# IvanPopov/video-flow-ml

Measured on AMD Instinct MI355X. Metric: flow-fields/sec @1080p seq5 MOF_sintel, higher is better.
Workload: dtype mixed (per-layer MFMA count, f32 accumulate): {"corr": 1, "update_block.encoder.convf1": 1, "update_block.encoder.convf2": 1, "update_block.gru.convq1.iter": "2a", "update_block.gru.convzr1.iter": 1, "update_block.gru.convzr2.iter": 1, "update_block.mask.0": 1, "update_block.mask.2": 1, "update_bloc

## Files before the change

video-flow-ml_amd/vfml/csrc/conv_gemm_split.hip:

```cpp
#include "conv_split_common.h"
#include "gemm_resident_walk.h"

namespace {

template <int BN, int WM, int WN, bool BIGC, bool IN16, int NM = 3>
__global__ __launch_bounds__(WM * WN * 64, 2) void conv_gemm_split_kernel(const SplitArgs a) {
  constexpr bool ALO = NM == 3 || NM == 2, BLO = NM == 3 || NM == 4;
  constexpr int NT = WM * WN * 64;
  constexpr int LR = NT / 4;
  constexpr int TM = BM / (WM * 32);
  constexpr int TN = BN / (WN * 32);
  constexpr int AU = BM / LR;
  constexpr int BU = BN / LR;
  constexpr int BUN = BU > 0 ? BU : 1;
  constexpr int RSA = BM + 2;
  constexpr int RSB = BN + 2;
  constexpr int SA = KG * RSA;
  constexpr int SB = KG * RSB;
  constexpr int LDC = BN + 4;

  extern __shared__ __attribute__((aligned(16))) char smem_raw[];
  h16x8* sAh = reinterpret_cast<h16x8*>(smem_raw);
  h16x8* sAl = sAh + 2 * SA;
  h16x8* sBh = sAl + 2 * SA;
// ... 154 lines not shown
    for (int j = 0; j < TN; ++j)
#pragma unroll
      for (int e = 0; e < 16; ++e) acc[i][j][e] = 0.f;

  auto compute = [&](int buf) {
    const int oa = buf * SA + wm * (BM / WM) + r;
    const int ob = buf * SB + wn * (BN / WN) + r;
#pragma unroll
    for (int ks = 0; ks < KG / 2; ++ks) {
      h16x8 ah[TM], al[TM], bh[TN], bl[TN];
#pragma unroll
      for (int i = 0; i < TM; ++i) {
        ah[i] = sAh[oa + (2 * ks + half) * RSA + i * 32];
        if constexpr (ALO) al[i] = sAl[oa + (2 * ks + half) * RSA + i * 32];
      }
#pragma unroll
      for (int j = 0; j < TN; ++j) {
        bh[j] = sBh[ob + (2 * ks + half) * RSB + j * 32];
        if constexpr (BLO) bl[j] = sBl[ob + (2 * ks + half) * RSB + j * 32];
      }
#pragma unroll
      for (int i = 0; i < TM; ++i)
#pragma unroll
        for (int j = 0; j < TN; ++j) {
          acc[i][j] = __builtin_amdgcn_mfma_f32_32x32x16_f16(ah[i], bh[j], acc[i][j], 0, 0, 0);
          if constexpr (BLO) acc[i][j] = __builtin_amdgcn_mfma_f32_32x32x16_f16(ah[i], bl[j], acc[i][j], 0, 0, 0);
          if constexpr (ALO) acc[i][j] = __builtin_amdgcn_mfma_f32_32x32x16_f16(al[i], bh[j], acc[i][j], 0, 0, 0);
        }
    }
  };

  const int nk = ((a.K + BK - 1) / BK + 1) & ~1;
  load_tile(st0, 0);
  load_tile(st1, BK);
  store_tile(st0, 0);
  __syncthreads();
  for (int kt = 0; kt < nk; kt += 2) {
    load_tile(st0, (kt + 2) * BK);
    __builtin_amdgcn_sched_barrier(0);
    compute(0);
    __builtin_amdgcn_sched_barrier(0);
    store_tile(st1, 1);
    __syncthreads();
    load_tile(st1, (kt + 3) * BK);
    __builtin_amdgcn_sched_barrier(0);
    compute(1);
    __builtin_amdgcn_sched_barrier(0);
    store_tile(st0, 0);
    __syncthreads();
  }

  acc_to_lds<TM, TN, LDC>(acc, sC, wm * (BM / WM), wn * (BN / WN), r, half);
  __syncthreads();
  if (!epilogue_rows_fast<BN, NT>(a, sC, m0, n0, t, BM, 32, 0)) epilogue_rows<BN, NT>(a, sC, m0, n0, t);
  if (a.stats_part) {
    constexpr int RG = NT / BN;
    const int ch = t % BN, rg = t / BN;
    double s1 = 0.0, s2 = 0.0;
    if (n0 + ch < a.cout) {
      const float b = a.bias ? a.bias[n0 + ch] : 0.f;
      for (int row = rg; row < BM; row += RG) {
        if (m0 + row >= a.M) break;
        const double v = (double)((sC[row * LDC + ch] * a.w_inv + b) * a.out_scale);
        s1 += v;
        s2 += v * v;
      }
    }
    __syncthreads();
    double* fold = reinterpret_cast<double*>(sC);
    fold[(rg * BN + ch) * 2] = s1;
    fold[(rg * BN + ch) * 2 + 1] = s2;
    __syncthreads();
    if (rg == 0 && n0 + ch < a.cout) {
      for (int g = 1; g < RG; ++g) {
        s1 += vfml_lds_f64(&fold[(g * BN + ch) * 2]);
        s2 += vfml_lds_f64(&fold[(g * BN + ch) * 2 + 1]);
      }
      double* o = a.stats_part + ((int64_t)(m0 / BM) * a.cout + n0 + ch) * 2;
      o[0] = s1;
      o[1] = s2;
    }
  }
}



template <int TM, int TN, int WM, int WN, bool PERSIST, bool FASTK, bool CSWAP = false, int NM = 3, bool MF16 = false, bool H16 = false>
__global__ __launch_bounds__(WM * WN * 64, (WM * WN == 4 ? 2 : 1)) void conv_gemm_dma_kernel(const SplitArgs a) {
  static_assert(!H16 || PERSIST, "VFML_FMT_F16 outputs (H16) exist in the persistent GEMM form only");
  static_assert(!(MF16 && PERSIST), "the persistent GEMM form runs 32x32x16 MFMAs (its 16x16x32 epilogue branches below are not maintained)");
  constexpr bool H64 = NM == 5;
  static_assert(!H64 || FASTK, "64-channel steps exist for the uniform-step loader only");
  constexpr bool BHI = NM == 2 || NM == 1 || H64;
  constexpr bool AHI = NM == 4 || NM == 1 || H64;
  constexpr int KSTEP = H64 ? 64 : BK;
  constexpr int NW = WM * WN, NT = NW * 64;
  constexpr int TBM = 32 * TM * WM, TBN = 32 * TN * WN;
  constexpr int AP = TBM / (8 * NW), BP = TBN / (8 * NW);
  static_assert(TBM % (8 * NW) == 0 && TBN % (8 * NW) == 0, "tile rows must split into whole pieces per wave");
  constexpr int ASZ = TBM * 128, BSZ = TBN * 128, STG = ASZ + BSZ;
  constexpr int LDC = TBN + 4;

  extern __shared__ __attribute__((aligned(16))) char smem_raw[];
  float* sC = reinterpret_cast<float*>(smem_raw);

  if constexpr (PERSIST && FASTK && !CSWAP && NM == 5 && !MF16) {
    if (a.resident) {
// ... 419 lines not shown
          }
        }
        if constexpr (PERSIST && TN == 2 && FASTK) if (a.out_t) {
          if constexpr (MF16) {
            static_for<2>([&](auto tc) {
              constexpr int t2 = decltype(tc)::value;
              static_for<2 * TN>([&](auto jc) {
                constexpr int j = decltype(jc)::value;
#pragma unroll
                for (int e = 0; e < 4; ++e) {
                  float v = 0.f;
                  static_for<TM>([&](auto ii) { if (decltype(ii)::value == i) v = acc4[2 * decltype(ii)::value + t2][j][e]; });
                  const int row = t2 * 16 + 4 * u4 + e, col = j * 16 + r4;
                  ws[col * 32 + ((row + (col >> 1)) & 31)] = v;
                }
              });
            });
          } else {
#pragma unroll
          for (int j = 0; j < TN; ++j)
#pragma unroll
            for (int e = 0; e < 16; ++e) {
              const int row = (e & 3) + 8 * (e >> 2) + 4 * half, col = j * 32 + r;
              ws[col * 32 + ((row + (col >> 1)) & 31)] = acc[i][j][e];
            }
          }
          const int rows_t = cols_valid, cols_t = rows_valid;
          char* tbase_t = reinterpret_cast<char*>(cur_ks ? a.out_t_k1 : a.out_t) + ((int64_t)cur_n0 * a.ld_out_t + cur_m0) * ES;
          const __amdgpu_buffer_rsrc_t rt =
              __builtin_amdgcn_make_buffer_rsrc(tbase_t, 0, ((rows_t - 1) * a.ld_out_t + cols_t) * ES, 0x00020000);
          const int g = lane >> 3, cl = lane & 7;
#pragma unroll
          for (int pp = 0; pp < 8; ++pp) {
            const int c = pp * 8 + cl;
            f32x4 v;
#pragma unroll
            for (int k = 0; k < 4; ++k) v[k] = ws[c * 32 + ((4 * g + k + (c >> 1)) & 31)] * a.w_inv * a.out_scale;
            const int q0 = wm * (32 * TM) + i * 32 + 4 * g;
            const int trow = wn * WC + c;
            const bool ok = trow < rows_t && q0 < cols_t;
            if constexpr (H16) {
              const h16x2 p0 = {(_Float16)v[0], (_Float16)v[1]}, p1 = {(_Float16)v[2], (_Float16)v[3]};
              const u32x2 hv = {__builtin_bit_cast(unsigned, p0), __builtin_bit_cast(unsigned, p1)};
              __builtin_amdgcn_raw_buffer_store_b64(hv, rt, ok ? (trow * a.ld_out_t + q0) * 2 : OOB, 0, STORE_NT);
            } else {
              __builtin_amdgcn_raw_buffer_store_b128(__builtin_bit_cast(u32x4, v), rt,
                                                     ok ? (trow * a.ld_out_t + q0) * 4 : OOB, 0, STORE_NT);
            }
          }
        }
      }
      stores_behind = true;
    } else {
      {
      static_for<TM>([&](auto slab) {
        constexpr int i = decltype(slab)::value;
        __syncthreads();
        if constexpr (PROJ && i == 0) {
          if (a.proj_out) proj_weights_store(pw, smem_raw + proj_lds_off<TBN>(), t);
        }
        if constexpr (MF16) {
          static_for<2>([&](auto tc) {
            constexpr int t2 = decltype(tc)::value;
            static_for<2 * TN>([&](auto jc) {
              constexpr int j = decltype(jc)::value;
              f32x4 v = {0.f, 0.f, 0.f, 0.f};
              static_for<TM>([&](auto ii) { if (decltype(ii)::value == i) v = acc4[2 * decltype(ii)::value + t2][j]; });
              *reinterpret_cast<f32x4*>(&sC[(wm * 32 + t2 * 16 + r4) * LDC + wn * (32 * TN) + j * 16 + 4 * u4]) = v;
            });
          });
        } else {
#pragma unroll
        for (int j = 0; j < TN; ++j)
#pragma unroll
          for (int e = 0; e < 16; ++e) {
            const int row = wm * 32 + (e & 3) + 8 * (e >> 2) + 4 * half;
            const int col = wn * (32 * TN) + j * 32 + r;
            sC[row * LDC + col] = acc[i][j][e];
          }
        }
        __syncthreads();
        bool projected = false;
        if constexpr (PROJ) {
          if (a.proj_out) {
            epilogue_proj_slab<TBN, NT, NM == 4>(a, sC, cur_m0, cur_n0, t, WM * 32, 32 * TM, i * 32);
            projected = true;
          }
        }
        if (!projected && !epilogue_rows_fast<TBN, NT>(a, sC, cur_m0, cur_n0, t, WM * 32, 32 * TM, i * 32))
          epilogue_rows<TBN, NT>(a, sC, cur_m0, cur_n0, t, WM * 32, 32 * TM, i * 32);
        if (a.stats_part) {
          for (int p = t; p < TBN * WM; p += NT) {
            const int ch = p % TBN, wb = p / TBN;
            const int g0 = cur_m0 + wb * (32 * TM) + i * 32;
            if (cur_n0 + ch < a.cout && g0 < a.M) {
              const float b = a.bias ? a.bias[cur_n0 + ch] : 0.f;
              double s1 = 0.0, s2 = 0.0;
              for (int rr = 0; rr < 32; ++rr) {
                if (g0 + rr >= a.M) break;
                const double v = (double)((sC[(wb * 32 + rr) * LDC + ch] * a.w_inv + b) * a.out_scale);
                s1 += v;
                s2 += v * v;
              }
              double* o = a.stats_part + ((int64_t)(g0 >> 5) * a.cout + cur_n0 + ch) * 2;
              o[0] = s1;
              o[1] = s2;
            }
          }
        }
      });
      }
    }
    if (!PERSIST || next >= tile_end) break;
    tile = next;
  }
}


template <int TM, int TN, int WM, int WN, bool PERSIST, bool FASTK, bool CSWAP = false, int NM = 3, bool MF16 = false, bool H16 = false>
int launch_dma_k(SplitArgs& a, hipStream_t s) {
  constexpr int TBM = 32 * TM * WM, TBN = 32 * TN * WN;
  constexpr size_t stage = 2 * (size_t)(TBM + TBN) * 128;
  constexpr size_t slab = (size_t)WM * 32 * (TBN + 4) * 4;
  constexpr size_t lds = (PERSIST || stage > slab) ? stage : slab;
  static_assert(lds <= 160 * 1024, "LDS");
  a.mtiles = (a.M + TBM - 1) / TBM;
  a.ntiles = (a.cout + TBN - 1) / TBN;
  constexpr bool HAS_RESIDENT = PERSIST && FASTK && !CSWAP && NM == 5 && !MF16;
  constexpr size_t lds_resident = VFML_RESIDENT_LDS;
  if (const int rc = vfml_lds_cap(reinterpret_cast<const void*>(&conv_gemm_dma_kernel<TM, TN, WM, WN, PERSIST, FASTK, CSWAP, NM, MF16, H16>),
                                  (int)(HAS_RESIDENT && lds_resident > lds ? lds_resident : lds), "vfml_conv2d_split"))
    return rc;
  if (a.resident) {
    if (!HAS_RESIDENT) {
      vfml_set_error("vfml_conv2d_split: the plan asks for the resident-A walk of a kernel that has none");
      return 1;
    }
    a.mtiles = (a.M + 127) / 128;
    a.ntiles = (a.cout + 63) / 64;
    int64_t best = -1;
    for (int nc = 1; nc <= a.ntiles && nc <= 512; ++nc) {
      const int cl = (a.ntiles + nc - 1) / nc, runs = (a.ntiles + cl - 1) / cl;
      const int64_t cost = (((int64_t)a.mtiles * runs + 511) / 512) * (cl + 3);
      if (best < 0 || cost < best) {
        best = cost;
        a.res_cl = cl;
        a.res_nc = runs;
      }
    }
    const int64_t units = (int64_t)a.mtiles * a.res_nc;
    hipLaunchKernelGGL((conv_gemm_dma_kernel<TM, TN, WM, WN, PERSIST, FASTK, CSWAP, NM, MF16, H16>), dim3((int)(units > 512 ? 512 : units)),
                       dim3(WM * WN * 64), lds_resident, s, a);
    return vfml_check_launch("vfml_conv2d_split");
  }
  const int64_t total = (int64_t)a.mtiles * a.ntiles * (PERSIST ? a.ksplit : 1);
  const int64_t slots = 256 * (WM * WN == 4 ? 2 : 1);
  const int grid = (int)(PERSIST && total > slots ? slots : total);
  hipLaunchKernelGGL((conv_gemm_dma_kernel<TM, TN, WM, WN, PERSIST, FASTK, CSWAP, NM, MF16, H16>), dim3(grid), dim3(WM * WN * 64), lds, s, a);
  return vfml_check_launch("vfml_conv2d_split");
}

template <int BN, int WM, int WN, bool BIGC, bool IN16, int NM>
int launch_nm(SplitArgs& a, hipStream_t s) {
// ... 646 lines not shown
```

video-flow-ml_amd/vfml/csrc/conv_gemm_tapx.hip:

```cpp
#include "conv_split_common.h"

#ifndef VFML_TAPX_HOOKS
#define TAPX_HOOK_ENTRY()
#define TAPX_HOOK_KLOOP_BEGIN()
#define TAPX_HOOK_STEP_BEGIN(st)
#define TAPX_HOOK_STAMP(k)
#define TAPX_HOOK_STEP_END()
#define TAPX_HOOK_KLOOP_END(nsteps)
#define TAPX_HOOK_EXIT()
#endif

namespace {

template <int TM, int TN, int WM, int WN, int NM>
__global__ __launch_bounds__(256, 2) void conv_gemm_tapx_kernel(const SplitArgs a) {
  constexpr bool H64 = NM == 5;
  constexpr bool BHI = NM == 2 || NM == 1 || H64;
  constexpr bool AHI = NM == 4 || NM == 1 || H64;
  constexpr int KSTEP = H64 ? 64 : 32;
  constexpr int NT = 256;
  static_assert(WM * WN == 4, "four waves: two workgroups per CU");
  constexpr int TBM = 32 * TM * WM, TBN = 32 * TN * WN;
  constexpr int NPA = (TBM + VFML_TAPX_KWMAX - 1 + 7) / 8;
  constexpr int NPI = (NPA + 3) / 4;
// ... 127 lines not shown
      const int R0 = r4 + kx;
      const int swa = (R0 >> 1) & 7;
      const int aoffk = abuf + (wm * (32 * TM) + R0) * 128 + (H64 ? (u4 ^ swa) : ((2 * u4) ^ swz16(swa))) * 16;
      auto a_addr = [&](int i) { return (unsigned)(oxp[i] + kx) < (unsigned)a.W ? aoffk + i * 2048 : ZOFF; };
      h16x8 a0, a1;
      {
        const int ad = a_addr(0);
        a0 = *reinterpret_cast<const h16x8*>(smem_raw + ad);
        if constexpr (H64 || !AHI) a1 = *reinterpret_cast<const h16x8*>(smem_raw + (ad ^ X1));
      }
      __syncthreads();
      TAPX_HOOK_STAMP(1);
      __builtin_amdgcn_sched_barrier(0);
      static_for<2 * TM>([&](auto ic) {
        constexpr int i = decltype(ic)::value;
        h16x8 n0_, n1_;
        if constexpr (i + 1 < 2 * TM) {
          const int ad = a_addr(i + 1);
          n0_ = *reinterpret_cast<const h16x8*>(smem_raw + ad);
          if constexpr (H64 || !AHI) n1_ = *reinterpret_cast<const h16x8*>(smem_raw + (ad ^ X1));
        }
        static_for<2 * TN>([&](auto jc) {
          constexpr int j = decltype(jc)::value;
          acc4[i][j] = __builtin_amdgcn_mfma_f32_16x16x32_f16(b0[j], a0, acc4[i][j], 0, 0, 0);
          if constexpr (H64) {
            acc4[i][j] = __builtin_amdgcn_mfma_f32_16x16x32_f16(b1[j], a1, acc4[i][j], 0, 0, 0);
          } else {
            if constexpr (!BHI) acc4[i][j] = __builtin_amdgcn_mfma_f32_16x16x32_f16(b1[j], a0, acc4[i][j], 0, 0, 0);
            if constexpr (!AHI) acc4[i][j] = __builtin_amdgcn_mfma_f32_16x16x32_f16(b0[j], a1, acc4[i][j], 0, 0, 0);
          }
          constexpr int g = i * (2 * TN) + j;
          if constexpr (g < BP) {
            if (next_step) issue_b(g, st + 1);
          } else if constexpr (g < BP + ASLOTS) {
            const int ia = kx + (g - BP) * a.kw;
            if (next_stage && ia < NPI && 4 * ia + wave < NPA) issue_a(ia, nbuf, cbn, kyn);
          }
          __builtin_amdgcn_sched_barrier(0);
        });
        if constexpr (i + 1 < 2 * TM) {
          a0 = n0_;
          if constexpr (H64 || !AHI) a1 = n1_;
        }
      });
      TAPX_HOOK_STAMP(2);
      asm volatile("s_waitcnt vmcnt(0)" ::: "memory");
      TAPX_HOOK_STAMP(3);
      __syncthreads();
      TAPX_HOOK_STEP_END();
    }
  }

  TAPX_HOOK_KLOOP_END(nsteps);
#pragma unroll
  for (int i = 0; i < TM; ++i) {
    if (i) lds_barrier();
    static_for<2>([&](auto tc) {
      constexpr int t2 = decltype(tc)::value;
      static_for<2 * TN>([&](auto jc) {
        constexpr int j = decltype(jc)::value;
        f32x4 v = {0.f, 0.f, 0.f, 0.f};
        static_for<TM>([&](auto ii) { if (decltype(ii)::value == i) v = acc4[2 * decltype(ii)::value + t2][j]; });
        *reinterpret_cast<f32x4*>(&sC[(wm * 32 + t2 * 16 + r4) * LDC + wn * (32 * TN) + j * 16 + 4 * u4]) = v;
      });
    });
    lds_barrier();
    if (!epilogue_rows_fast<TBN, NT>(a, sC, m0, n0, t, WM * 32, 32 * TM, i * 32))
      epilogue_rows<TBN, NT>(a, sC, m0, n0, t, WM * 32, 32 * TM, i * 32);
    if (a.stats_part) {
      for (int p = t; p < TBN * WM; p += NT) {
        const int ch = p % TBN, wb = p / TBN;
        const int g0 = m0 + wb * (32 * TM) + i * 32;
        if (n0 + ch < a.cout && g0 < a.M) {
          const float b = a.bias ? a.bias[n0 + ch] : 0.f;
          double s1 = 0.0, s2 = 0.0;
          for (int rr = 0; rr < 32; ++rr) {
            if (g0 + rr >= a.M) break;
            const double v = (double)((sC[(wb * 32 + rr) * LDC + ch] * a.w_inv + b) * a.out_scale);
            s1 += v;
            s2 += v * v;
          }
          double* o = a.stats_part + ((int64_t)(g0 >> 5) * a.cout + n0 + ch) * 2;
          o[0] = s1;
          o[1] = s2;
        }
      }
    }
  }
  TAPX_HOOK_EXIT();
}

template <int TM, int TN, int WM, int WN, int NM>
int launch_tapx_k(SplitArgs& a, hipStream_t s) {
  constexpr int TBM = 32 * TM * WM, TBN = 32 * TN * WN;
  constexpr int NPA = (TBM + VFML_TAPX_KWMAX - 1 + 7) / 8;
  constexpr size_t stage = 2 * (size_t)NPA * 1024 + (size_t)TBN * 128 + 128;
  constexpr size_t slab = (size_t)WM * 32 * (TBN + 4) * 4;
  constexpr size_t lds = stage > slab ? stage : slab;
  static_assert(lds <= 80 * 1024, "two workgroups per CU");
  a.mtiles = (a.M + TBM - 1) / TBM;
  a.ntiles = (a.cout + TBN - 1) / TBN;
  if (const int rc = vfml_lds_cap(reinterpret_cast<const void*>(&conv_gemm_tapx_kernel<TM, TN, WM, WN, NM>), (int)lds,
                                  "vfml_conv2d_split"))
    return rc;
  hipLaunchKernelGGL((conv_gemm_tapx_kernel<TM, TN, WM, WN, NM>), dim3(a.mtiles * a.ntiles), dim3(256), lds, s, a);
  return vfml_check_launch("vfml_conv2d_split");
}

#define TAPX_ROWS(TM, TN, WM, WN) \
  {vfml_detail::tapx_plan(TM, TN, WM, WN, 3), &launch_tapx_k<TM, TN, WM, WN, 3>}, \
  {vfml_detail::tapx_plan(TM, TN, WM, WN, 5), &launch_tapx_k<TM, TN, WM, WN, 5>}
const SplitVariant TAPX_VARIANTS[] = {TAPX_ROWS(3, 2, 2, 2), TAPX_ROWS(2, 3, 2, 2), TAPX_ROWS(2, 2, 4, 1), TAPX_ROWS(2, 3, 4, 1)};
#undef TAPX_ROWS

}

const SplitVariant* vfml_detail::tapx_variant(const SplitPlan& plan) {
  return find_variant(TAPX_VARIANTS, sizeof(TAPX_VARIANTS) / sizeof(TAPX_VARIANTS[0]), plan);
}

const SplitVariant* vfml_detail::tapx_variant_at(int index) {
  const int n = (int)(sizeof(TAPX_VARIANTS) / sizeof(TAPX_VARIANTS[0]));
  return index >= 0 && index < n ? &TAPX_VARIANTS[index] : nullptr;
}
```

video-flow-ml_amd/vfml/csrc/conv_split_common.h:

```cpp
#pragma once
#include <hip/hip_fp16.h>
#include <stdlib.h>
#include <utility>
#include "vfml_common.h"


namespace vfml_detail {
struct SplitArgs {
  const float* in0; const float* in1;
  const _Float16* whi; const _Float16* wlo; const float* bias;
  const float* aux0; const float* aux1; const float* addend;
  float* out;
  int c0, ld0, c1, ld1, ctot, ld_addend;
  int H, W, ho, wo;
  int kh, kw, stride, pad_h, pad_w;
  int M, K, Kp, cout;
  int d0off, d1off;
  int bytes0, bytesw;
  int ldo, ld_aux0, ld_aux1;
  int epilogue, split;
  float out_scale, w_inv;
  int mtiles, ntiles;
  int vec_ok;
  int out16, aux16;
// ... 189 lines not shown
      if (nvalid == 4) {
        if (epi == VFML_EPI_GRU_ZR && !lowhalf) x0 = aux4(a.aux0, a.ld_aux0, grow, col - a.split);
        if (epi == VFML_EPI_GRU_Q) {
          x0 = aux4(a.aux0, a.ld_aux0, grow, col);
          x1 = aux4(a.aux1, a.ld_aux1, grow, col);
        }
        if (epi == VFML_EPI_ADD_AUX) x0 = aux4(a.aux0, a.ld_aux0, grow, col);
      } else {
        for (int e = 0; e < nvalid; ++e) {
          if (epi == VFML_EPI_GRU_ZR && !lowhalf) x0[e] = a.aux0[(int64_t)grow * a.ld_aux0 + col + e - a.split];
          if (epi == VFML_EPI_GRU_Q) {
            x0[e] = a.aux0[(int64_t)grow * a.ld_aux0 + col + e];
            x1[e] = a.aux1[(int64_t)grow * a.ld_aux1 + col + e];
          }
          if (epi == VFML_EPI_ADD_AUX) x0[e] = a.aux0[(int64_t)grow * a.ld_aux0 + col + e];
        }
      }
#pragma unroll
      for (int e = 0; e < 4; ++e) v[e] = epi1(v[e], epi, lowhalf, x0[e], x1[e]);
      if (a.out16) {
        U8 hi, lo;
        split4(v, hi, lo, 0);
        char* u = reinterpret_cast<char*>(a.out + (int64_t)grow * a.ldo + gcol) + 8 * q;
        *reinterpret_cast<uint2*>(u) = __builtin_bit_cast(uint2, __builtin_shufflevector(hi.v, hi.v, 0, 1, 2, 3));
        *reinterpret_cast<uint2*>(u + 16) = __builtin_bit_cast(uint2, __builtin_shufflevector(lo.v, lo.v, 0, 1, 2, 3));
      } else {
        float* o = a.out + (int64_t)grow * a.ldo + col;
        if (nvalid == 4 && a.vec_ok) {
          *reinterpret_cast<f32x4*>(o) = v;
        } else {
          for (int e = 0; e < nvalid; ++e) o[e] = v[e];
        }
      }
    }
  }
}

template <int EPI>
__device__ __forceinline__ void epi_unit(f32x4 (&v)[2], const f32x4 (&x0)[2], const f32x4 (&x1)[2], bool lowhalf) {
#pragma unroll
  for (int q = 0; q < 2; ++q)
#pragma unroll
    for (int e = 0; e < 4; ++e) {
      float r = v[q][e];
      if constexpr (EPI == VFML_EPI_RELU) r = fmaxf(r, 0.f);
      else if constexpr (EPI == VFML_EPI_TANH) r = tanhf(r);
      else if constexpr (EPI == VFML_EPI_SIGMOID) r = sigmoidf_(r);
      else if constexpr (EPI == VFML_EPI_GRU_ZR) { r = sigmoidf_(r); r = lowhalf ? r : r * x0[q][e]; }
      else if constexpr (EPI == VFML_EPI_GRU_Q) r = (1.f - x0[q][e]) * x1[q][e] + x0[q][e] * tanhf(r);
      v[q][e] = r;
    }
}

__device__ __forceinline__ void load_unit16(const float* base, int64_t off, f32x4 (&x)[2]) {
  const h16x8 h = *reinterpret_cast<const h16x8*>(base + off);
  const h16x8 l = *reinterpret_cast<const h16x8*>(base + off + 4);
#pragma unroll
  for (int e = 0; e < 8; ++e) x[e >> 2][e & 3] = (float)h[e] + (float)l[e];
}

template <int BN, int NT, int EPI>
__device__ __forceinline__ void epilogue_rows_fast_k(const SplitArgs& a, const float* sC, int m0, int n0, int t, int nrows,
                                                     int rstride, int roff) {
  constexpr int LDC = BN + 4;
  constexpr int C8 = BN / 8;
  constexpr int RPP = NT / C8;
  if constexpr (NT % C8 != 0) {
    if (t >= RPP * C8) return;
  }
  const int c8 = t % C8;
  const int gcol = n0 + c8 * 8;
  if (gcol >= a.cout) return;
  const bool whole = gcol + 8 <= a.cout;
  f32x4 bias4[2] = {{0.f, 0.f, 0.f, 0.f}, {0.f, 0.f, 0.f, 0.f}};
  if (a.bias) {
    bias4[0] = *reinterpret_cast<const f32x4*>(a.bias + gcol);
    if (whole) bias4[1] = *reinterpret_cast<const f32x4*>(a.bias + gcol + 4);
  }
  const bool lowhalf = gcol < a.split;
  const vfml_gfptr addend = addend_of(a);
  struct RowOps {
    f32x4 add[2], x0[2], x1[2];
  };
  auto load_row = [&](int row, RowOps& o) {
    const int grow = m0 + (row >> 5) * rstride + roff + (row & 31);
    o.add[0] = o.add[1] = f32x4{0.f, 0.f, 0.f, 0.f};
    o.x0[0] = o.x0[1] = o.x1[0] = o.x1[1] = f32x4{0.f, 0.f, 0.f, 0.f};
    if (row >= nrows || grow >= a.M) return;
    if (a.addend) {
      o.add[0] = *(vfml_gf4ptr)(addend + (int64_t)grow * a.ld_addend + gcol);
      if (whole) o.add[1] = *(vfml_gf4ptr)(addend + (int64_t)grow * a.ld_addend + gcol + 4);
    }
    if constexpr (EPI == VFML_EPI_GRU_ZR) {
      if (!lowhalf) load_unit16(a.aux0, (int64_t)grow * a.ld_aux0 + gcol - a.split, o.x0);
    }
    if constexpr (EPI == VFML_EPI_GRU_Q) {
      load_unit16(a.aux0, (int64_t)grow * a.ld_aux0 + gcol, o.x0);
      load_unit16(a.aux1, (int64_t)grow * a.ld_aux1 + gcol, o.x1);
    }
  };
  constexpr int EB = EPI == VFML_EPI_GRU_Q ? 2 : 4;
  for (int row0 = t / C8; row0 < nrows; row0 += EB * RPP) {
    RowOps ops[EB];
    static_for<EB>([&](auto bc) { load_row(row0 + decltype(bc)::value * RPP, ops[decltype(bc)::value]); });
    static_for<EB>([&](auto bc) {
      constexpr int b = decltype(bc)::value;
      const int row = row0 + b * RPP;
      const int grow = m0 + (row >> 5) * rstride + roff + (row & 31);
      if (row < nrows && grow < a.M) {
        const RowOps& cur = ops[b];
        f32x4 v[2];
        v[0] = *reinterpret_cast<const f32x4*>(&sC[row * LDC + c8 * 8]);
        v[1] = *reinterpret_cast<const f32x4*>(&sC[row * LDC + c8 * 8 + 4]);
#pragma unroll
        for (int q = 0; q < 2; ++q)
#pragma unroll
          for (int e = 0; e < 4; ++e) v[q][e] = (v[q][e] * a.w_inv + cur.add[q][e] + bias4[q][e]) * a.out_scale;
        epi_unit<EPI>(v, cur.x0, cur.x1, lowhalf);
        if (a.out16) {
          U8 hi, lo;
          split4(v[0], hi, lo, 0);
          split4(v[1], hi, lo, 4);
          float* u = a.out + (int64_t)grow * a.ldo + gcol;
          if (whole) {
            *reinterpret_cast<h16x8*>(u) = hi.v;
            *reinterpret_cast<h16x8*>(u + 4) = lo.v;
          } else {
            *reinterpret_cast<uint2*>(u) = __builtin_bit_cast(uint2, __builtin_shufflevector(hi.v, hi.v, 0, 1, 2, 3));
            *reinterpret_cast<uint2*>(u + 4) = __builtin_bit_cast(uint2, __builtin_shufflevector(lo.v, lo.v, 0, 1, 2, 3));
          }
        } else {
          float* o = a.out + (int64_t)grow * a.ldo + gcol;
          *reinterpret_cast<f32x4*>(o) = v[0];
          if (whole) *reinterpret_cast<f32x4*>(o + 4) = v[1];
        }
      }
    });
  }
}

__device__ __forceinline__ void lds_barrier() {
#if defined(__HIP_DEVICE_COMPILE__)
  asm volatile("s_waitcnt lgkmcnt(0)\n\ts_barrier" ::: "memory");
#endif
}

constexpr int PROJ_ROW = 272, PROJ_ROWS = 48, PROJ_PIECES = 2 * PROJ_ROWS * 16 / 256;
template <int BN>
constexpr int proj_lds_off() { return 64 * (BN + 4) * 4; }
__device__ __forceinline__ void proj_weights_load(const SplitArgs& a, int n0, int t, u32x4 (&pw)[PROJ_PIECES]) {
  const __amdgpu_buffer_rsrc_t rw = __builtin_amdgcn_make_buffer_rsrc(const_cast<char*>(a.proj_w), 0, a.proj_bytes, 0x00020000);
  static_for<PROJ_PIECES>([&](auto kc) {
    constexpr int k = decltype(kc)::value;
    const int q = t + 256 * k, plane = q / (PROJ_ROWS * 16), rem = q % (PROJ_ROWS * 16), n = rem >> 4, seg = rem & 15;
    const int off = n < a.proj_n ? (n * a.proj_kp + n0) * 2 + seg * 16 : (int)0x40000000;
    pw[k] = __builtin_bit_cast(u32x4, __builtin_amdgcn_raw_buffer_load_b128(rw, off, plane ? a.proj_lo_off : 0, 0));
  });
}
__device__ __forceinline__ void proj_weights_store(const u32x4 (&pw)[PROJ_PIECES], char* lds, int t) {
  static_for<PROJ_PIECES>([&](auto kc) {
    constexpr int k = decltype(kc)::value;
    const int q = t + 256 * k, plane = q / (PROJ_ROWS * 16), rem = q % (PROJ_ROWS * 16), n = rem >> 4, seg = rem & 15;
    *reinterpret_cast<u32x4*>(lds + (plane * PROJ_ROWS + n) * PROJ_ROW + seg * 16) = pw[k];
  });
}

template <int BN, int NT, bool AHI>
__device__ __forceinline__ void epilogue_proj_slab(const SplitArgs& a, float* sC, int m0, int n0, int t, int nrows, int rstride,
                                                   int roff) {
  static_assert(BN == 128 && NT == 256, "projection epilogue: 128-column tiles of four waves");
  constexpr int LDC = BN + 4, C8 = BN / 8, RPP = NT / C8;
  const int c8 = t % C8;
  const int gcol = n0 + c8 * 8;
  f32x4 bias4[2] = {{0.f, 0.f, 0.f, 0.f}, {0.f, 0.f, 0.f, 0.f}};
  if (a.bias && gcol < a.cout) {
    bias4[0] = *reinterpret_cast<const f32x4*>(a.bias + gcol);
    bias4[1] = *reinterpret_cast<const f32x4*>(a.bias + gcol + 4);
  }
  for (int row = t / C8; row < nrows; row += RPP) {
    float* u = &sC[row * LDC + c8 * 8];
    f32x4 v[2] = {*reinterpret_cast<const f32x4*>(u), *reinterpret_cast<const f32x4*>(u + 4)};
#pragma unroll
    for (int q = 0; q < 2; ++q)
#pragma unroll
      for (int e = 0; e < 4; ++e) v[q][e] = fmaxf((v[q][e] * a.w_inv + bias4[q][e]) * a.out_scale, 0.f);
    if (gcol >= a.cout) v[0] = v[1] = f32x4{0.f, 0.f, 0.f, 0.f};
    U8 hi, lo;
    split4(v[0], hi, lo, 0);
    split4(v[1], hi, lo, 4);
    *reinterpret_cast<h16x8*>(u) = hi.v;
    *reinterpret_cast<h16x8*>(u + 4) = lo.v;
  }
  lds_barrier();
  const int lane = t & 63, wave = t >> 6;
  const int r = lane & 15, g = lane >> 4;
  f32x4 d[3] = {{0.f, 0.f, 0.f, 0.f}, {0.f, 0.f, 0.f, 0.f}, {0.f, 0.f, 0.f, 0.f}};
  const char* arow = reinterpret_cast<const char*>(sC) + (16 * wave + r) * (LDC * 4) + g * 32;
  const char* brow = reinterpret_cast<const char*>(sC) + proj_lds_off<BN>() + r * PROJ_ROW + g * 16;
  static_for<4>([&](auto sc) {
    constexpr int ks = decltype(sc)::value;
    h16x8 bh[3], bl[3];
#pragma unroll
    for (int j = 0; j < 3; ++j) {
      bh[j] = *reinterpret_cast<const h16x8*>(brow + 16 * j * PROJ_ROW + ks * 64);
      bl[j] = *reinterpret_cast<const h16x8*>(brow + (PROJ_ROWS + 16 * j) * PROJ_ROW + ks * 64);
    }
    const h16x8 ah = *reinterpret_cast<const h16x8*>(arow + ks * 128);
    h16x8 al;
    if constexpr (!AHI) al = *reinterpret_cast<const h16x8*>(arow + ks * 128 + 16);
#pragma unroll
    for (int j = 0; j < 3; ++j) {
      d[j] = __builtin_amdgcn_mfma_f32_16x16x32_f16(bh[j], ah, d[j], 0, 0, 0);
      d[j] = __builtin_amdgcn_mfma_f32_16x16x32_f16(bl[j], ah, d[j], 0, 0, 0);
      if constexpr (!AHI) d[j] = __builtin_amdgcn_mfma_f32_16x16x32_f16(bh[j], al, d[j], 0, 0, 0);
    }
  });
  const int srow = 16 * wave + r;
  const int grow = m0 + (srow >> 5) * rstride + roff + (srow & 31);
  if (srow < nrows && grow < a.M) {
    float* o = a.proj_out + ((int64_t)(n0 / BN) * a.M + grow) * a.ld_proj;
#pragma unroll
    for (int j = 0; j < 3; ++j) {
      const int n = 16 * j + 4 * g;
      if (n < a.proj_n) {
        f32x4 v = d[j];
#pragma unroll
        for (int e = 0; e < 4; ++e) v[e] *= a.proj_inv;
        *reinterpret_cast<f32x4*>(o + n) = v;
      }
    }
  }
}

template <int BN, int NT>
__device__ __forceinline__ bool epilogue_rows_fast(const SplitArgs& a, const float* sC, int m0, int n0, int t, int nrows,
                                                   int rstride, int roff) {
  const bool gru = a.epilogue == VFML_EPI_GRU_ZR || a.epilogue == VFML_EPI_GRU_Q;
  if (!(a.vec_ok && a.cout % 4 == 0 && (!gru || (a.aux16 && a.split % 8 == 0 && a.cout % 8 == 0)) &&
        (!a.bias || (reinterpret_cast<uintptr_t>(a.bias) & 15u) == 0) && a.epilogue != VFML_EPI_TANH_RELU &&
        a.epilogue != VFML_EPI_ADD_AUX))
    return false;
  switch (a.epilogue) {
    case VFML_EPI_NONE: epilogue_rows_fast_k<BN, NT, VFML_EPI_NONE>(a, sC, m0, n0, t, nrows, rstride, roff); return true;
    case VFML_EPI_RELU: epilogue_rows_fast_k<BN, NT, VFML_EPI_RELU>(a, sC, m0, n0, t, nrows, rstride, roff); return true;
    case VFML_EPI_GRU_ZR: epilogue_rows_fast_k<BN, NT, VFML_EPI_GRU_ZR>(a, sC, m0, n0, t, nrows, rstride, roff); return true;
    case VFML_EPI_GRU_Q: epilogue_rows_fast_k<BN, NT, VFML_EPI_GRU_Q>(a, sC, m0, n0, t, nrows, rstride, roff); return true;
    default: return false;
  }
}

typedef __attribute__((address_space(3))) void* lds_ptr_t;

__device__ __forceinline__ void dma16(__amdgpu_buffer_rsrc_t rsrc, int voff_bytes, int soff_bytes, char* lds) {
#if defined(__HIP_DEVICE_COMPILE__)
  __builtin_amdgcn_raw_ptr_buffer_load_lds(rsrc, (lds_ptr_t)lds, 16, voff_bytes, soff_bytes, 0, 0);
#endif
}

__device__ __forceinline__ constexpr int swz16(int x) { return x ^ ((((x >> 1) ^ (x >> 2)) & 1) << 1); }

}
```

Before: 49.57.

## Software-pipeline epilogue global loads across slabs with compile-time row counts

Restructures the GEMM conv epilogue into a FastRows helper that issues the addend/aux loads for the next row batch (and the next slab) before finishing the current one. This hides global-load latency behind LDS reads and stores. The row count becomes a compile-time template parameter, and the epilogue kind is dispatched once per tile instead of per slab. Intermediate syncthreads are replaced with lighter lds_barrier calls. The cost is more register pressure from double-buffered RowOps and more template instantiations.

```diff
diff --git a/video-flow-ml_amd/vfml/csrc/conv_gemm_split.hip b/video-flow-ml_amd/vfml/csrc/conv_gemm_split.hip
--- a/video-flow-ml_amd/vfml/csrc/conv_gemm_split.hip
+++ b/video-flow-ml_amd/vfml/csrc/conv_gemm_split.hip
@@ -230,7 +230,7 @@
 
   acc_to_lds<TM, TN, LDC>(acc, sC, wm * (BM / WM), wn * (BN / WN), r, half);
   __syncthreads();
-  if (!epilogue_rows_fast<BN, NT>(a, sC, m0, n0, t, BM, 32, 0)) epilogue_rows<BN, NT>(a, sC, m0, n0, t);
+  if (!epilogue_rows_fast<BN, NT, BM>(a, sC, m0, n0, t, 32, 0)) epilogue_rows<BN, NT>(a, sC, m0, n0, t);
   if (a.stats_part) {
     constexpr int RG = NT / BN;
     const int ch = t % BN, rg = t / BN;
@@ -756,11 +756,20 @@
       }
       stores_behind = true;
     } else {
-      {
+      auto slabs = [&](auto kind) {
+      constexpr int KIND = decltype(kind)::value;
+      using Rows = FastRows<TBN, NT, KIND < 0 ? VFML_EPI_NONE : KIND, WM * 32, TM == 3 ? 2 : 4>;
+      Rows rows;
+      typename Rows::RowOps ops[2][Rows::EB];
+      if constexpr (KIND >= 0) {
+        rows.begin(a, cur_n0, t);
+        rows.request(a, cur_m0, 32 * TM, 0, 0, ops[0]);
+      }
       static_for<TM>([&](auto slab) {
         constexpr int i = decltype(slab)::value;
-        __syncthreads();
-        if constexpr (PROJ && i == 0) {
+        if constexpr (i == 0) __syncthreads();
+        else lds_barrier();
+        if constexpr (PROJ && i == 0 && KIND < 0) {
           if (a.proj_out) proj_weights_store(pw, smem_raw + proj_lds_off<TBN>(), t);
         }
         if constexpr (MF16) {
@@ -783,16 +792,20 @@
             sC[row * LDC + col] = acc[i][j][e];
           }
         }
-        __syncthreads();
-        bool projected = false;
-        if constexpr (PROJ) {
-          if (a.proj_out) {
-            epilogue_proj_slab<TBN, NT, NM == 4>(a, sC, cur_m0, cur_n0, t, WM * 32, 32 * TM, i * 32);
-            projected = true;
+        lds_barrier();
+        if constexpr (KIND >= 0) {
+          fast_rows_slab<TM, i>(rows, ops, a, sC, cur_m0);
+        } else {
+          bool projected = false;
+          if constexpr (PROJ) {
+            if (a.proj_out) {
+              epilogue_proj_slab<TBN, NT, NM == 4>(a, sC, cur_m0, cur_n0, t, WM * 32, 32 * TM, i * 32);
+              projected = true;
+            }
           }
+          if (!projected) epilogue_rows<TBN, NT>(a, sC, cur_m0, cur_n0, t, WM * 32, 32 * TM, i * 32);
         }
-        if (!projected && !epilogue_rows_fast<TBN, NT>(a, sC, cur_m0, cur_n0, t, WM * 32, 32 * TM, i * 32))
-          epilogue_rows<TBN, NT>(a, sC, cur_m0, cur_n0, t, WM * 32, 32 * TM, i * 32);
+        if constexpr (KIND < 0 || KIND == VFML_EPI_NONE) {
         if (a.stats_part) {
           for (int p = t; p < TBN * WM; p += NT) {
             const int ch = p % TBN, wb = p / TBN;
@@ -812,7 +825,17 @@
             }
           }
         }
+        }
       });
+      };
+      bool proj_call = false;
+      if constexpr (PROJ) proj_call = a.proj_out != nullptr;
+      switch (proj_call ? -1 : fast_rows_kind(a)) {
+        case VFML_EPI_NONE: slabs(std::integral_constant<int, VFML_EPI_NONE>{}); break;
+        case VFML_EPI_RELU: slabs(std::integral_constant<int, VFML_EPI_RELU>{}); break;
+        case VFML_EPI_GRU_ZR: slabs(std::integral_constant<int, VFML_EPI_GRU_ZR>{}); break;
+        case VFML_EPI_GRU_Q: slabs(std::integral_constant<int, VFML_EPI_GRU_Q>{}); break;
+        default: slabs(std::integral_constant<int, -1>{}); break;
       }
     }
     if (!PERSIST || next >= tile_end) break;
diff --git a/video-flow-ml_amd/vfml/csrc/conv_gemm_tapx.hip b/video-flow-ml_amd/vfml/csrc/conv_gemm_tapx.hip
--- a/video-flow-ml_amd/vfml/csrc/conv_gemm_tapx.hip
+++ b/video-flow-ml_amd/vfml/csrc/conv_gemm_tapx.hip
@@ -203,40 +203,57 @@
   }
 
   TAPX_HOOK_KLOOP_END(nsteps);
-#pragma unroll
-  for (int i = 0; i < TM; ++i) {
-    if (i) lds_barrier();
-    static_for<2>([&](auto tc) {
-      constexpr int t2 = decltype(tc)::value;
-      static_for<2 * TN>([&](auto jc) {
-        constexpr int j = decltype(jc)::value;
-        f32x4 v = {0.f, 0.f, 0.f, 0.f};
-        static_for<TM>([&](auto ii) { if (decltype(ii)::value == i) v = acc4[2 * decltype(ii)::value + t2][j]; });
-        *reinterpret_cast<f32x4*>(&sC[(wm * 32 + t2 * 16 + r4) * LDC + wn * (32 * TN) + j * 16 + 4 * u4]) = v;
+  auto slabs = [&](auto kind) {
+    constexpr int KIND = decltype(kind)::value;
+    using Rows = FastRows<TBN, NT, KIND < 0 ? VFML_EPI_NONE : KIND, WM * 32, TM == 3 ? 2 : 4>;
+    Rows rows;
+    typename Rows::RowOps ops[2][Rows::EB];
+    if constexpr (KIND >= 0) {
+      rows.begin(a, n0, t);
+      rows.request(a, m0, 32 * TM, 0, 0, ops[0]);
+    }
+    static_for<TM>([&](auto slab) {
+      constexpr int i = decltype(slab)::value;
+      if constexpr (i > 0) lds_barrier();
+      static_for<2>([&](auto tc) {
+        constexpr int t2 = decltype(tc)::value;
+        static_for<2 * TN>([&](auto jc) {
+          constexpr int j = decltype(jc)::value;
+          *reinterpret_cast<f32x4*>(&sC[(wm * 32 + t2 * 16 + r4) * LDC + wn * (32 * TN) + j * 16 + 4 * u4]) = acc4[2 * i + t2][j];
+        });
       });
+      lds_barrier();
+      if constexpr (KIND >= 0) fast_rows_slab<TM, i>(rows, ops, a, sC, m0);
+      else epilogue_rows<TBN, NT>(a, sC, m0, n0, t, WM * 32, 32 * TM, i * 32);
+      if constexpr (KIND < 0 || KIND == VFML_EPI_NONE) {
+        if (a.stats_part) {
+          for (int p = t; p < TBN * WM; p += NT) {
+            const int ch = p % TBN, wb = p / TBN;
+            const int g0 = m0 + wb * (32 * TM) + i * 32;
+            if (n0 + ch < a.cout && g0 < a.M) {
+              const float b = a.bias ? a.bias[n0 + ch] : 0.f;
+              double s1 = 0.0, s2 = 0.0;
+              for (int rr = 0; rr < 32; ++rr) {
+                if (g0 + rr >= a.M) break;
+                const double v = (double)((sC[(wb * 32 + rr) * LDC + ch] * a.w_inv + b) * a.out_scale);
+                s1 += v;
+                s2 += v * v;
+              }
+              double* o = a.stats_part + ((int64_t)(g0 >> 5) * a.cout + n0 + ch) * 2;
+              o[0] = s1;
+              o[1] = s2;
+            }
+          }
+        }
+      }
     });
-    lds_barrier();
-    if (!epilogue_rows_fast<TBN, NT>(a, sC, m0, n0, t, WM * 32, 32 * TM, i * 32))
-      epilogue_rows<TBN, NT>(a, sC, m0, n0, t, WM * 32, 32 * TM, i * 32);
-    if (a.stats_part) {
-      for (int p = t; p < TBN * WM; p += NT) {
-        const int ch = p % TBN, wb = p / TBN;
-        const int g0 = m0 + wb * (32 * TM) + i * 32;
-        if (n0 + ch < a.cout && g0 < a.M) {
-          const float b = a.bias ? a.bias[n0 + ch] : 0.f;
-          double s1 = 0.0, s2 = 0.0;
-          for (int rr = 0; rr < 32; ++rr) {
-            if (g0 + rr >= a.M) break;
-            const double v = (double)((sC[(wb * 32 + rr) * LDC + ch] * a.w_inv + b) * a.out_scale);
-            s1 += v;
-            s2 += v * v;
-          }
-          double* o = a.stats_part + ((int64_t)(g0 >> 5) * a.cout + n0 + ch) * 2;
-          o[0] = s1;
-          o[1] = s2;
-        }
-      }
-    }
+  };
+  switch (fast_rows_kind(a)) {
+    case VFML_EPI_NONE: slabs(std::integral_constant<int, VFML_EPI_NONE>{}); break;
+    case VFML_EPI_RELU: slabs(std::integral_constant<int, VFML_EPI_RELU>{}); break;
+    case VFML_EPI_GRU_ZR: slabs(std::integral_constant<int, VFML_EPI_GRU_ZR>{}); break;
+    case VFML_EPI_GRU_Q: slabs(std::integral_constant<int, VFML_EPI_GRU_Q>{}); break;
+    default: slabs(std::integral_constant<int, -1>{}); break;
   }
   TAPX_HOOK_EXIT();
 }
diff --git a/video-flow-ml_amd/vfml/csrc/conv_split_common.h b/video-flow-ml_amd/vfml/csrc/conv_split_common.h
--- a/video-flow-ml_amd/vfml/csrc/conv_split_common.h
+++ b/video-flow-ml_amd/vfml/csrc/conv_split_common.h
@@ -265,91 +265,162 @@
     }
 }
 
-__device__ __forceinline__ void load_unit16(const float* base, int64_t off, f32x4 (&x)[2]) {
-  const h16x8 h = *reinterpret_cast<const h16x8*>(base + off);
-  const h16x8 l = *reinterpret_cast<const h16x8*>(base + off + 4);
-#pragma unroll
-  for (int e = 0; e < 8; ++e) x[e >> 2][e & 3] = (float)h[e] + (float)l[e];
-}
-
-template <int BN, int NT, int EPI>
-__device__ __forceinline__ void epilogue_rows_fast_k(const SplitArgs& a, const float* sC, int m0, int n0, int t, int nrows,
-                                                     int rstride, int roff) {
-  constexpr int LDC = BN + 4;
-  constexpr int C8 = BN / 8;
-  constexpr int RPP = NT / C8;
-  if constexpr (NT % C8 != 0) {
-    if (t >= RPP * C8) return;
-  }
-  const int c8 = t % C8;
-  const int gcol = n0 + c8 * 8;
-  if (gcol >= a.cout) return;
-  const bool whole = gcol + 8 <= a.cout;
-  f32x4 bias4[2] = {{0.f, 0.f, 0.f, 0.f}, {0.f, 0.f, 0.f, 0.f}};
-  if (a.bias) {
-    bias4[0] = *reinterpret_cast<const f32x4*>(a.bias + gcol);
-    if (whole) bias4[1] = *reinterpret_cast<const f32x4*>(a.bias + gcol + 4);
-  }
-  const bool lowhalf = gcol < a.split;
-  const vfml_gfptr addend = addend_of(a);
+template <int BN, int NT, int EPI, int ROWS, int EBMAX = 4>
+struct FastRows {
+  static constexpr int LDC = BN + 4;
+  static constexpr int C8 = BN / 8;
+  static constexpr int RPP = NT / C8;
+  static constexpr int NR = (ROWS + RPP - 1) / RPP;
+  static constexpr int EB0 = EPI == VFML_EPI_GRU_Q || C8 != 16 ? 2 : EBMAX;
+  static constexpr int EB = EB0 < NR ? EB0 : NR;
+  static constexpr int NB = (NR + EB - 1) / EB;
   struct RowOps {
-    f32x4 add[2], x0[2], x1[2];
+    f32x4 add[2];
+    h16x8 h0, l0, h1, l1;
   };
-  auto load_row = [&](int row, RowOps& o) {
-    const int grow = m0 + (row >> 5) * rstride + roff + (row & 31);
-    o.add[0] = o.add[1] = f32x4{0.f, 0.f, 0.f, 0.f};
-    o.x0[0] = o.x0[1] = o.x1[0] = o.x1[1] = f32x4{0.f, 0.f, 0.f, 0.f};
-    if (row >= nrows || grow >= a.M) return;
-    if (a.addend) {
-      o.add[0] = *(vfml_gf4ptr)(addend + (int64_t)grow * a.ld_addend + gcol);
-      if (whole) o.add[1] = *(vfml_gf4ptr)(addend + (int64_t)grow * a.ld_addend + gcol + 4);
-    }
-    if constexpr (EPI == VFML_EPI_GRU_ZR) {
-      if (!lowhalf) load_unit16(a.aux0, (int64_t)grow * a.ld_aux0 + gcol - a.split, o.x0);
-    }
-    if constexpr (EPI == VFML_EPI_GRU_Q) {
-      load_unit16(a.aux0, (int64_t)grow * a.ld_aux0 + gcol, o.x0);
-      load_unit16(a.aux1, (int64_t)grow * a.ld_aux1 + gcol, o.x1);
-    }
-  };
-  constexpr int EB = EPI == VFML_EPI_GRU_Q ? 2 : 4;
-  for (int row0 = t / C8; row0 < nrows; row0 += EB * RPP) {
-    RowOps ops[EB];
-    static_for<EB>([&](auto bc) { load_row(row0 + decltype(bc)::value * RPP, ops[decltype(bc)::value]); });
+  bool live;
+  bool whole, lowhalf;
+  int c8, gcol, trow;
+  f32x4 bias4[2];
+  vfml_gfptr addend;
+
+  __device__ __forceinline__ void begin(const SplitArgs& a, int n0, int t) {
+    c8 = t % C8;
+    trow = t / C8;
+    gcol = n0 + c8 * 8;
+    live = gcol < a.cout;
+    if constexpr (NT % C8 != 0) live = live && t < RPP * C8;
+    whole = gcol + 8 <= a.cout;
+    lowhalf = gcol < a.split;
+    bias4[0] = bias4[1] = f32x4{0.f, 0.f, 0.f, 0.f};
+    addend = nullptr;
+    if (!live) return;
+    if (a.bias) {
+      bias4[0] = *reinterpret_cast<const f32x4*>(a.bias + gcol);
+      if (whole) bias4[1] = *reinterpret_cast<const f32x4*>(a.bias + gcol + 4);
+    }
+    addend = addend_of(a);
+  }
+
+  __device__ __forceinline__ void request(const SplitArgs& a, int m0, int rstride, int roff, int batch, RowOps (&ops)[EB]) const {
+    if (!live) return;
     static_for<EB>([&](auto bc) {
-      constexpr int b = decltype(bc)::value;
-      const int row = row0 + b * RPP;
+      RowOps& o = ops[decltype(bc)::value];
+      const int row = trow + (batch * EB + decltype(bc)::value) * RPP;
       const int grow = m0 + (row >> 5) * rstride + roff + (row & 31);
-      if (row < nrows && grow < a.M) {
-        const RowOps& cur = ops[b];
-        f32x4 v[2];
-        v[0] = *reinterpret_cast<const f32x4*>(&sC[row * LDC + c8 * 8]);
-        v[1] = *reinterpret_cast<const f32x4*>(&sC[row * LDC + c8 * 8 + 4]);
-#pragma unroll
-        for (int q = 0; q < 2; ++q)
-#pragma unroll
-          for (int e = 0; e < 4; ++e) v[q][e] = (v[q][e] * a.w_inv + cur.add[q][e] + bias4[q][e]) * a.out_scale;
-        epi_unit<EPI>(v, cur.x0, cur.x1, lowhalf);
-        if (a.out16) {
-          U8 hi, lo;
-          split4(v[0], hi, lo, 0);
-          split4(v[1], hi, lo, 4);
-          float* u = a.out + (int64_t)grow * a.ldo + gcol;
-          if (whole) {
-            *reinterpret_cast<h16x8*>(u) = hi.v;
-            *reinterpret_cast<h16x8*>(u + 4) = lo.v;
-          } else {
-            *reinterpret_cast<uint2*>(u) = __builtin_bit_cast(uint2, __builtin_shufflevector(hi.v, hi.v, 0, 1, 2, 3));
-            *reinterpret_cast<uint2*>(u + 4) = __builtin_bit_cast(uint2, __builtin_shufflevector(lo.v, lo.v, 0, 1, 2, 3));
-          }
+      if (row >= ROWS || grow >= a.M) return;
+      if (a.addend) {
+        o.add[0] = *(vfml_gf4ptr)(addend + (int64_t)grow * a.ld_addend + gcol);
+        if (whole) o.add[1] = *(vfml_gf4ptr)(addend + (int64_t)grow * a.ld_addend + gcol + 4);
+      }
+      if constexpr (EPI == VFML_EPI_GRU_ZR) {
+        if (!lowhalf) {
+          o.h0 = *reinterpret_cast<const h16x8*>(a.aux0 + (int64_t)grow * a.ld_aux0 + gcol - a.split);
+          o.l0 = *reinterpret_cast<const h16x8*>(a.aux0 + (int64_t)grow * a.ld_aux0 + gcol - a.split + 4);
+        }
+      }
+      if constexpr (EPI == VFML_EPI_GRU_Q) {
+        o.h0 = *reinterpret_cast<const h16x8*>(a.aux0 + (int64_t)grow * a.ld_aux0 + gcol);
+        o.l0 = *reinterpret_cast<const h16x8*>(a.aux0 + (int64_t)grow * a.ld_aux0 + gcol + 4);
+        o.h1 = *reinterpret_cast<const h16x8*>(a.aux1 + (int64_t)grow * a.ld_aux1 + gcol);
+        o.l1 = *reinterpret_cast<const h16x8*>(a.aux1 + (int64_t)grow * a.ld_aux1 + gcol + 4);
+      }
+    });
+  }
+
+  __device__ __forceinline__ void finish(const SplitArgs& a, const float* sC, int m0, int rstride, int roff, int batch,
+                                         const RowOps (&ops)[EB]) const {
+    if (!live) return;
+    static_for<EB>([&](auto bc) {
+      const RowOps& cur = ops[decltype(bc)::value];
+      const int row = trow + (batch * EB + decltype(bc)::value) * RPP;
+      const int grow = m0 + (row >> 5) * rstride + roff + (row & 31);
+      if (row >= ROWS || grow >= a.M) return;
+      const f32x4 zero = {0.f, 0.f, 0.f, 0.f};
+      f32x4 add[2] = {zero, zero}, x0[2] = {zero, zero}, x1[2] = {zero, zero};
+      if (a.addend) {
+        add[0] = cur.add[0];
+        if (whole) add[1] = cur.add[1];
+      }
+      if constexpr (EPI == VFML_EPI_GRU_ZR) {
+        if (!lowhalf) {
+#pragma unroll
+          for (int e = 0; e < 8; ++e) x0[e >> 2][e & 3] = (float)cur.h0[e] + (float)cur.l0[e];
+        }
+      }
+      if constexpr (EPI == VFML_EPI_GRU_Q) {
+#pragma unroll
+        for (int e = 0; e < 8; ++e) {
+          x0[e >> 2][e & 3] = (float)cur.h0[e] + (float)cur.l0[e];
+          x1[e >> 2][e & 3] = (float)cur.h1[e] + (float)cur.l1[e];
+        }
+      }
+      f32x4 v[2];
+      v[0] = *reinterpret_cast<const f32x4*>(&sC[row * LDC + c8 * 8]);
+      v[1] = *reinterpret_cast<const f32x4*>(&sC[row * LDC + c8 * 8 + 4]);
+#pragma unroll
+      for (int q = 0; q < 2; ++q)
+#pragma unroll
+        for (int e = 0; e < 4; ++e) v[q][e] = (v[q][e] * a.w_inv + add[q][e] + bias4[q][e]) * a.out_scale;
+      epi_unit<EPI>(v, x0, x1, lowhalf);
+      if (a.out16) {
+        U8 hi, lo;
+        split4(v[0], hi, lo, 0);
+        split4(v[1], hi, lo, 4);
+        float* u = a.out + (int64_t)grow * a.ldo + gcol;
+        if (whole) {
+          *reinterpret_cast<h16x8*>(u) = hi.v;
+          *reinterpret_cast<h16x8*>(u + 4) = lo.v;
         } else {
-          float* o = a.out + (int64_t)grow * a.ldo + gcol;
-          *reinterpret_cast<f32x4*>(o) = v[0];
-          if (whole) *reinterpret_cast<f32x4*>(o + 4) = v[1];
-        }
+          *reinterpret_cast<uint2*>(u) = __builtin_bit_cast(uint2, __builtin_shufflevector(hi.v, hi.v, 0, 1, 2, 3));
+          *reinterpret_cast<uint2*>(u + 4) = __builtin_bit_cast(uint2, __builtin_shufflevector(lo.v, lo.v, 0, 1, 2, 3));
+        }
+      } else {
+        float* o = a.out + (int64_t)grow * a.ldo + gcol;
+        *reinterpret_cast<f32x4*>(o) = v[0];
+        if (whole) *reinterpret_cast<f32x4*>(o + 4) = v[1];
       }
     });
   }
+};
+
+__device__ __forceinline__ int fast_rows_kind(const SplitArgs& a) {
+  const bool gru = a.epilogue == VFML_EPI_GRU_ZR || a.epilogue == VFML_EPI_GRU_Q;
+  if (!(a.vec_ok && a.cout % 4 == 0 && (!gru || (a.aux16 && a.split % 8 == 0 && a.cout % 8 == 0)) &&
+        (!a.bias || (reinterpret_cast<uintptr_t>(a.bias) & 15u) == 0)))
+    return -1;
+  switch (a.epilogue) {
+    case VFML_EPI_NONE:
+    case VFML_EPI_RELU:
+    case VFML_EPI_GRU_ZR:
+    case VFML_EPI_GRU_Q: return a.epilogue;
+    default: return -1;
+  }
+}
+
+template <int TM, int I, class Rows>
+__device__ __forceinline__ void fast_rows_slab(const Rows& rows, typename Rows::RowOps (&ops)[2][Rows::EB], const SplitArgs& a,
+                                               const float* sC, int m0) {
+  static_for<Rows::NB>([&](auto bc) {
+    constexpr int k = I * Rows::NB + decltype(bc)::value, kn = k + 1;
+    if constexpr (kn < TM * Rows::NB) rows.request(a, m0, 32 * TM, (kn / Rows::NB) * 32, kn % Rows::NB, ops[kn & 1]);
+    rows.finish(a, sC, m0, 32 * TM, I * 32, k % Rows::NB, ops[k & 1]);
+  });
+}
+
+template <int BN, int NT, int EPI, int ROWS>
+__device__ __forceinline__ void epilogue_rows_fast_k(const SplitArgs& a, const float* sC, int m0, int n0, int t, int rstride,
+                                                     int roff) {
+  using Rows = FastRows<BN, NT, EPI, ROWS>;
+  Rows rows;
+  typename Rows::RowOps ops[2][Rows::EB];
+  rows.begin(a, n0, t);
+  rows.request(a, m0, rstride, roff, 0, ops[0]);
+  static_for<Rows::NB>([&](auto bc) {
+    constexpr int b = decltype(bc)::value;
+    if constexpr (b + 1 < Rows::NB) rows.request(a, m0, rstride, roff, b + 1, ops[(b + 1) & 1]);
+    rows.finish(a, sC, m0, rstride, roff, b, ops[b & 1]);
+  });
 }
 
 __device__ __forceinline__ void lds_barrier() {
@@ -445,19 +516,14 @@
   }
 }
 
-template <int BN, int NT>
-__device__ __forceinline__ bool epilogue_rows_fast(const SplitArgs& a, const float* sC, int m0, int n0, int t, int nrows,
-                                                   int rstride, int roff) {
-  const bool gru = a.epilogue == VFML_EPI_GRU_ZR || a.epilogue == VFML_EPI_GRU_Q;
-  if (!(a.vec_ok && a.cout % 4 == 0 && (!gru || (a.aux16 && a.split % 8 == 0 && a.cout % 8 == 0)) &&
-        (!a.bias || (reinterpret_cast<uintptr_t>(a.bias) & 15u) == 0) && a.epilogue != VFML_EPI_TANH_RELU &&
-        a.epilogue != VFML_EPI_ADD_AUX))
-    return false;
-  switch (a.epilogue) {
-    case VFML_EPI_NONE: epilogue_rows_fast_k<BN, NT, VFML_EPI_NONE>(a, sC, m0, n0, t, nrows, rstride, roff); return true;
-    case VFML_EPI_RELU: epilogue_rows_fast_k<BN, NT, VFML_EPI_RELU>(a, sC, m0, n0, t, nrows, rstride, roff); return true;
-    case VFML_EPI_GRU_ZR: epilogue_rows_fast_k<BN, NT, VFML_EPI_GRU_ZR>(a, sC, m0, n0, t, nrows, rstride, roff); return true;
-    case VFML_EPI_GRU_Q: epilogue_rows_fast_k<BN, NT, VFML_EPI_GRU_Q>(a, sC, m0, n0, t, nrows, rstride, roff); return true;
+template <int BN, int NT, int ROWS>
+__device__ __forceinline__ bool epilogue_rows_fast(const SplitArgs& a, const float* sC, int m0, int n0, int t, int rstride,
+                                                   int roff) {
+  switch (fast_rows_kind(a)) {
+    case VFML_EPI_NONE: epilogue_rows_fast_k<BN, NT, VFML_EPI_NONE, ROWS>(a, sC, m0, n0, t, rstride, roff); return true;
+    case VFML_EPI_RELU: epilogue_rows_fast_k<BN, NT, VFML_EPI_RELU, ROWS>(a, sC, m0, n0, t, rstride, roff); return true;
+    case VFML_EPI_GRU_ZR: epilogue_rows_fast_k<BN, NT, VFML_EPI_GRU_ZR, ROWS>(a, sC, m0, n0, t, rstride, roff); return true;
+    case VFML_EPI_GRU_Q: epilogue_rows_fast_k<BN, NT, VFML_EPI_GRU_Q, ROWS>(a, sC, m0, n0, t, rstride, roff); return true;
     default: return false;
   }
 }
```

New measurement: 49.81, median of 6. Within noise of the previous version (+0.5%).
